# CogSP/CoEvoNet

Hardware: AMD Instinct MI355X
Metric: env-steps/sec (agent-steps of the whole job; generations/sec in gens_per_sec), Co-GA simple_adversary_v3 pop=200 HoF=5 (higher is better)
Workload: dtype f32

## Files before the change

### coevonet_amd/csrc/coevo_common.hip.h

```cpp
#pragma once
#include <hip/hip_runtime.h>
#include <stdint.h>

#include "../../include/coevo.h"

namespace coevo {

constexpr int H1 = COEVO_FC_H1;
constexpr int H2 = COEVO_FC_H2;
constexpr int NACT = COEVO_FC_NACT;
constexpr float LN_EPS = 1e-5f;

__host__ __device__ constexpr int64_t fc_off_b1(int D) { return (int64_t)D * H1; }
__host__ __device__ constexpr int64_t fc_off_w2(int D) { return fc_off_b1(D) + 3 * H1; }
__host__ __device__ constexpr int64_t fc_off_b2(int D) { return fc_off_w2(D) + (int64_t)H1 * H2; }
__host__ __device__ constexpr int64_t fc_off_w3(int D) { return fc_off_b2(D) + 3 * H2; }
__host__ __device__ constexpr int64_t fc_off_b3(int D) { return fc_off_w3(D) + NACT * H2; }
__host__ __device__ constexpr int64_t fc_params(int D) { return fc_off_b3(D) + NACT; }
__host__ __device__ constexpr int64_t fc_stride(int D) { return (fc_params(D) + 63) / 64 * 64; }
__host__ __device__ constexpr int64_t fc_off_g1(int D) { return fc_off_b1(D) + H1; }
__host__ __device__ constexpr int64_t fc_off_g2(int D) { return fc_off_b2(D) + H2; }
__host__ __device__ inline bool fc_slab_is_layernorm(int64_t s, int D)
{
    const int64_t g1 = fc_off_g1(D), g2 = fc_off_g2(D);
// ... 157 lines not shown
{
    const size_t N = (size_t)n;
    s.ax = st[0 * N + g]; s.ay = st[1 * N + g];
    s.bx = st[2 * N + g]; s.by = st[3 * N + g];
    s.cx = st[4 * N + g]; s.cy = st[5 * N + g];
    s.avx = st[6 * N + g]; s.avy = st[7 * N + g];
    s.bvx = st[8 * N + g]; s.bvy = st[9 * N + g];
    s.cvx = st[10 * N + g]; s.cvy = st[11 * N + g];
    s.l0x = st[12 * N + g]; s.l0y = st[13 * N + g];
    s.l1x = st[14 * N + g]; s.l1y = st[15 * N + g];
    s.gx = st[16 * N + g]; s.gy = st[17 * N + g];
}

__device__ __forceinline__ void mpe_store_game(double *st, int n, int g, const MpeGame &s)
{
    const size_t N = (size_t)n;
    st[0 * N + g] = s.ax; st[1 * N + g] = s.ay;
    st[2 * N + g] = s.bx; st[3 * N + g] = s.by;
    st[4 * N + g] = s.cx; st[5 * N + g] = s.cy;
    st[6 * N + g] = s.avx; st[7 * N + g] = s.avy;
    st[8 * N + g] = s.bvx; st[9 * N + g] = s.bvy;
    st[10 * N + g] = s.cvx; st[11 * N + g] = s.cvy;
    st[12 * N + g] = s.l0x; st[13 * N + g] = s.l0y;
    st[14 * N + g] = s.l1x; st[15 * N + g] = s.l1y;
    st[16 * N + g] = s.gx; st[17 * N + g] = s.gy;
}

__device__ __forceinline__ void mpe_move(double &pos, double &vel, double u, int pos_first)
{
    const double f = (((u * 5.0) + 0.0) / 1.0) * 0.1;
    if (pos_first) pos = pos + vel * 0.1;
    vel = vel * 0.75;
    vel = vel + f;
    if (!pos_first) pos = pos + vel * 0.1;
}

__device__ __forceinline__ double mpe_ux(int act) { return act == 1 ? -1.0 : (act == 2 ? 1.0 : 0.0); }
__device__ __forceinline__ double mpe_uy(int act) { return act == 3 ? -1.0 : (act == 4 ? 1.0 : 0.0); }

__device__ __forceinline__ void mpe_world_move(MpeGame &s, int act_a, int act_b, int act_c, int pos_first)
{
    mpe_move(s.ax, s.avx, mpe_ux(act_a), pos_first);
    mpe_move(s.ay, s.avy, mpe_uy(act_a), pos_first);
    mpe_move(s.bx, s.bvx, mpe_ux(act_b), pos_first);
    mpe_move(s.by, s.bvy, mpe_uy(act_b), pos_first);
    mpe_move(s.cx, s.cvx, mpe_ux(act_c), pos_first);
    mpe_move(s.cy, s.cvy, mpe_uy(act_c), pos_first);
}

__device__ __forceinline__ void mpe_world_step(MpeGame &s, int act_a, int act_b, int act_c, int pos_first,
                                               double &r_good, double &r_adv)
{
    mpe_world_move(s, act_a, act_b, act_c, pos_first);
    double dx = s.ax - s.gx, dy = s.ay - s.gy;
    const double da = sqrt(dx * dx + dy * dy);
    dx = s.bx - s.gx; dy = s.by - s.gy;
    const double db = sqrt(dx * dx + dy * dy);
    dx = s.cx - s.gx; dy = s.cy - s.gy;
    const double dc = sqrt(dx * dx + dy * dy);
    r_adv = -da;
    const double m = (dc < db) ? dc : db;
    r_good = -m + da;
}

__host__ __device__ __forceinline__ void mpe_obs_good(const MpeGame &s, double mex, double mey, double ox, double oy, float o[10])
{
    o[0] = (float)(s.gx - mex);  o[1] = (float)(s.gy - mey);
    o[2] = (float)(s.l0x - mex); o[3] = (float)(s.l0y - mey);
    o[4] = (float)(s.l1x - mex); o[5] = (float)(s.l1y - mey);
    o[6] = (float)(s.ax - mex);  o[7] = (float)(s.ay - mey);
    o[8] = (float)(ox - mex);    o[9] = (float)(oy - mey);
}

__host__ __device__ __forceinline__ void mpe_obs_from_game(const MpeGame &s, int slot, float o[10])
{
    if (slot == COEVO_SLOT_ADVERSARY) {
        o[0] = (float)(s.l0x - s.ax); o[1] = (float)(s.l0y - s.ay);
        o[2] = (float)(s.l1x - s.ax); o[3] = (float)(s.l1y - s.ay);
        o[4] = (float)(s.bx - s.ax);  o[5] = (float)(s.by - s.ay);
        o[6] = (float)(s.cx - s.ax);  o[7] = (float)(s.cy - s.ay);
        o[8] = 0.0f;                  o[9] = 0.0f;
    } else if (slot == COEVO_SLOT_AGENT_0) {
        mpe_obs_good(s, s.bx, s.by, s.cx, s.cy, o);
    } else {
        mpe_obs_good(s, s.cx, s.cy, s.bx, s.by, o);
    }
}

__device__ __forceinline__ void mpe_fused_observe(const double *st_prev, double *st_next, const int32_t *act_prev,
                                         const int32_t *game_limit, int n, int g, int slot, int cycle, int pos_first,
                                         float *obs_out)
{
    const size_t N = (size_t)n;
    MpeGame s;
    mpe_load_game(st_prev, n, g, s);
    if (cycle > 0) {
        const int limit = game_limit ? game_limit[g] : 0x7fffffff;
        const int t0 = 3 * (cycle - 1);
        const bool stepped = t0 + 2 < limit;
        double r_good = 0.0, r_adv = 0.0;
        if (stepped) {
            const int a0 = act_prev[3 * g], a1 = act_prev[3 * g + 1], a2 = act_prev[3 * g + 2];
            if (slot == COEVO_SLOT_ADVERSARY) mpe_world_step(s, a0, a1, a2, pos_first, r_good, r_adv);
            else mpe_world_move(s, a0, a1, a2, pos_first);
        }
        if (slot == COEVO_SLOT_ADVERSARY) {
            double rg_prev = st_prev[18 * N + g], a_adv = st_prev[19 * N + g], a_a0 = st_prev[20 * N + g],
                   a_a1 = st_prev[21 * N + g];
            if (t0 < limit) a_adv = a_adv + rg_prev;
            if (t0 + 1 < limit) a_a0 = a_a0 + rg_prev;
            if (stepped) { a_a1 = a_a1 + r_adv; rg_prev = r_good; }
            mpe_store_game(st_next, n, g, s);
            st_next[18 * N + g] = rg_prev;
            st_next[19 * N + g] = a_adv;
            st_next[20 * N + g] = a_a0;
            st_next[21 * N + g] = a_a1;
        }
    }
    mpe_obs_from_game(s, slot, obs_out);
}

__device__ inline double block_sum_f64(double v, double *scratch)
{
#pragma unroll
    for (int m = 1; m < 64; m <<= 1) v = v + __shfl_xor(v, m, 64);
    const int w = threadIdx.x >> 6;
    if ((threadIdx.x & 63) == 0) scratch[w] = v;
    __syncthreads();
    const double tot = ((scratch[0] + scratch[1]) + scratch[2]) + scratch[3];
    __syncthreads();
    return tot;
}

template <class DistOf>
__device__ inline double sharing_row_total(DistOf dist_of, int n, double *scratch)
{
    double s = 0.0;
    for (int i = threadIdx.x; i < n; i += 256) s += (double)dist_of(i);
    const float sigma = (float)(block_sum_f64(s, scratch) / (double)n);
    double sc = 0.0;
    for (int i = threadIdx.x; i < n; i += 256) {
        const float sh = 1.0f - dist_of(i) / sigma;
        if (!(sh <= 0.0f)) sc += (double)sh;
    }
    return block_sum_f64(sc, scratch);
}

__device__ inline float ga_fitness_value(double reward, int hof, float share)
{
    const float total = (float)(reward / (double)hof);
    return total / (1.0f + share);
}

__device__ __forceinline__ double wave_sum_partials(const double *partial, int n_blocks)
{
    double v = 0.0;
    for (int b = threadIdx.x; b < n_blocks; b += 64) v += partial[b];
#pragma unroll
    for (int m = 1; m < 64; m <<= 1) v = v + __shfl_xor(v, m, 64);
    return v;
}

__device__ inline bool bad_post_relu(float y) { return __builtin_isnan(y) || (__builtin_isinf(y) && y > 0.0f); }
__device__ inline float relu_keep_nan(float y) { return !(y <= 0.0f) ? y : 0.0f; }

}

#ifndef COEVO_TU_FLAGS
#define COEVO_TU_FLAGS ""
#endif
#define COEVO_DEFINE_TU_FLAGS(tu) \
    namespace coevo { const char *tu_flags_##tu() { return COEVO_TU_FLAGS; } }

#define COEVO_HIP_CHECK(expr)                        \
    do {                                             \
        hipError_t _e = (expr);                      \
        if (_e != hipSuccess) return COEVO_ERR_HIP;  \
    } while (0)
```

### coevonet_amd/csrc/mpe_env.hip

```cpp
#include "coevo_common.hip.h"

#include "../../include/coevo_crossplay.h"

namespace coevo {

typedef unsigned __int128 u128;

__host__ __device__ inline u128 pcg_mult()
{
    return (((u128)0x2360ED051FC65DA4ULL) << 64) | (u128)0x4385DF649FCCF645ULL;
}

__host__ __device__ inline uint64_t pcg_output(u128 s)
{
    const uint64_t hi = (uint64_t)(s >> 64), lo = (uint64_t)s;
    const uint64_t x = hi ^ lo;
    const unsigned r = (unsigned)(hi >> 58);
    return (x >> r) | (x << ((64 - r) & 63));
}

__host__ __device__ inline u128 pcg_advance(u128 state, u128 inc, u128 delta)
{
    u128 acc_mult = 1, acc_plus = 0, cur_mult = pcg_mult(), cur_plus = inc;
    while (delta > 0) {
        if (delta & 1) {
            acc_mult *= cur_mult;
            acc_plus = acc_plus * cur_mult + cur_plus;
        }
        cur_plus = (cur_mult + 1) * cur_plus;
        cur_mult *= cur_mult;
        delta >>= 1;
    }
    return acc_mult * state + acc_plus;
}

__host__ __device__ __forceinline__ void mpe_reset_game(double *st, int n, int g, coevo_pcg64 rng, uint64_t ordinal);

__global__ void mpe_reset_kernel(double *st, int n, int game_first, int count, coevo_pcg64 rng,
                                 int64_t first_ordinal, const int32_t *gen_dev, int64_t ordinals_per_gen, int unsigned_first)
{
    const int i = blockIdx.x * blockDim.x + threadIdx.x;
    if (i >= count) return;
    int64_t first = first_ordinal + (gen_dev ? (int64_t)(*gen_dev) * ordinals_per_gen : 0);
    if (first < 0 && !unsigned_first) first = 0;
    mpe_reset_game(st, n, game_first + i, rng, (uint64_t)first + (uint64_t)i);
}

__global__ void mpe_reset_episodes_kernel(double *st, int n, int game_first, int count, coevo_pcg64 rng,
                                          uint64_t first_ordinal, int episodes)
{
    const int i = blockIdx.x * blockDim.x + threadIdx.x;
    if (i >= count) return;
    mpe_reset_game(st, n, game_first + i, rng, first_ordinal + (uint64_t)(i % episodes));
}

static_assert(sizeof(coevo_reset_seg) == 16, "layout mirrored by coevonet_amd/lib.py ResetSeg");
struct ResetSegs { coevo_reset_seg s[COEVO_MAX_JOBS]; };
__global__ void mpe_reset_multi_kernel(double *st, int n, ResetSegs segs, coevo_pcg64 rng, uint64_t *stamps, int n_stamps,
                                       int32_t *zero_words, int n_zero)
{
    const coevo_reset_seg &sg = segs.s[blockIdx.y];
    const int i = blockIdx.x * blockDim.x + threadIdx.x;
    if (zero_words && blockIdx.y == gridDim.y - 1)
        for (int j = i; j < n_zero; j += gridDim.x * blockDim.x) zero_words[j] = 0;
    if (stamps && blockIdx.y == 0)
        for (int j = i; j < n_stamps; j += gridDim.x * blockDim.x) {
            stamps[2 * j] = ~0ull;
            stamps[2 * j + 1] = 0ull;
        }
    if (i >= sg.count) return;
    mpe_reset_game(st, n, sg.game_first + i, rng, sg.first_ordinal + (uint64_t)i);
}

__host__ __device__ __forceinline__ void mpe_reset_game(double *st, int n, int g, coevo_pcg64 rng, uint64_t ordinal)
{
    const u128 inc = ((u128)rng.pcg_inc_hi << 64) | rng.pcg_inc_lo;
    u128 s = ((u128)rng.pcg_state_hi << 64) | rng.pcg_state_lo;
    s = pcg_advance(s, inc, (u128)(ordinal >> 1) * 21);
    s = s * pcg_mult() + inc;
    const uint64_t c = pcg_output(s);
    const uint32_t half = (ordinal & 1) ? (uint32_t)(c >> 32) : (uint32_t)c;
    const int goal = (int)(((uint64_t)half * 2) >> 32);
    if (ordinal & 1) s = pcg_advance(s, inc, 10);
    double d[10];
#pragma unroll
    for (int i = 0; i < 10; ++i) {
        s = s * pcg_mult() + inc;
        d[i] = -1.0 + 2.0 * ((double)(pcg_output(s) >> 11) * (1.0 / 9007199254740992.0));
    }
    const size_t N = (size_t)n;
#pragma unroll
    for (int i = 0; i < 6; ++i) {
        st[i * N + g] = d[i];
        st[(6 + i) * N + g] = 0.0;
    }
#pragma unroll
    for (int i = 0; i < 4; ++i) st[(12 + i) * N + g] = d[6 + i];
    st[16 * N + g] = d[6 + 2 * goal];
    st[17 * N + g] = d[7 + 2 * goal];
    st[18 * N + g] = 0.0;
    st[19 * N + g] = 0.0;
    st[20 * N + g] = 0.0;
    st[21 * N + g] = 0.0;
    st[22 * N + g] = (double)goal;
    st[23 * N + g] = 0.0;
}

__host__ __device__ inline float mpe_observe_at(const double *st, int n, const int32_t *row_game, const int32_t *row_slot, int i)
{
    const int row = i / COEVO_OBS_STRIDE, k = i % COEVO_OBS_STRIDE;
    const int slot = row_slot[row];
    const int D = (slot == COEVO_SLOT_ADVERSARY) ? 8 : 10;
    return (k < D) ? mpe_obs_element(st, n, row_game[row], slot, k) : 0.0f;
}

__global__ void mpe_observe_kernel(const double *st, int n, const int32_t *row_game, const int32_t *row_slot,
                                   int n_rows, float *obs)
{
    const int i = blockIdx.x * blockDim.x + threadIdx.x;
    if (i >= n_rows * COEVO_OBS_STRIDE) return;
    obs[i] = mpe_observe_at(st, n, row_game, row_slot, i);
}

__host__ __device__ inline void mpe_step_game(double *st, int n, const int32_t *game_rows, const int32_t *actions,
                                              int cycle, const int32_t *game_limit, int pos_first, int g)
{
    const size_t N = (size_t)n;
    const int limit = game_limit ? game_limit[g] : 0x7fffffff;
    const int t0 = 3 * cycle;
    if (t0 >= limit) return;
    const double rg_prev = st[18 * N + g];
    st[19 * N + g] = st[19 * N + g] + rg_prev;
    if (t0 + 1 < limit) st[20 * N + g] = st[20 * N + g] + rg_prev;
    if (t0 + 2 >= limit) return;
    double d[3];
    const double gx = st[16 * N + g], gy = st[17 * N + g];
#pragma unroll
    for (int i = 0; i < 3; ++i) {
        const int act = actions[game_rows[3 * g + i]];
        double u[2] = {0.0, 0.0};
        if (act == 1) u[0] = -1.0;
        if (act == 2) u[0] = +1.0;
        if (act == 3) u[1] = -1.0;
        if (act == 4) u[1] = +1.0;
        double p[2];
#pragma unroll
        for (int c = 0; c < 2; ++c) {
            const double f = (((u[c] * 5.0) + 0.0) / 1.0) * 0.1;
            double pos = st[(2 * i + c) * N + g], vel = st[(6 + 2 * i + c) * N + g];
            if (pos_first) pos = pos + vel * 0.1;
            vel = vel * 0.75;
            vel = vel + f;
            if (!pos_first) pos = pos + vel * 0.1;
            st[(2 * i + c) * N + g] = pos;
            st[(6 + 2 * i + c) * N + g] = vel;
            p[c] = pos;
        }
        const double dx = p[0] - gx, dy = p[1] - gy;
        d[i] = sqrt(dx * dx + dy * dy);
    }
    const double r_adv = -d[0];
    const double m = (d[2] < d[1]) ? d[2] : d[1];
    const double r_good = -m + d[0];
    st[21 * N + g] = st[21 * N + g] + r_adv;
    st[18 * N + g] = r_good;
}

__global__ void mpe_step_kernel(double *st, int n, const int32_t *game_rows, const int32_t *actions, int cycle,
                                const int32_t *game_limit, int pos_first)
{
    const int g = blockIdx.x * blockDim.x + threadIdx.x;
    if (g < n) mpe_step_game(st, n, game_rows, actions, cycle, game_limit, pos_first, g);
}

typedef coevo_final_pack FinalPack;
static_assert(sizeof(coevo_final_pack) == 40, "layout mirrored by coevonet_amd/lib.py FinalPack");

__global__ void mpe_final_step_kernel(const double *st, int n, const int32_t *act, int cycle,
                                      const int32_t *game_limit, int pos_first, double *rewards, FinalPack pk)
{
    const int g = blockIdx.x * blockDim.x + threadIdx.x;
    if (g >= n) return;
    const size_t N = (size_t)n;
    double a_adv = st[19 * N + g], a_a0 = st[20 * N + g], a_a1 = st[21 * N + g];
    if (cycle >= 0) {
        const int limit = game_limit ? game_limit[g] : 0x7fffffff;
        const int t0 = 3 * cycle;
        const double rg_prev = st[18 * N + g];
        if (t0 < limit) a_adv = a_adv + rg_prev;
        if (t0 + 1 < limit) a_a0 = a_a0 + rg_prev;
        if (t0 + 2 < limit) {
            MpeGame s;
            mpe_load_game(st, n, g, s);
            double r_good, r_adv;
            mpe_world_step(s, act[3 * g], act[3 * g + 1], act[3 * g + 2], pos_first, r_good, r_adv);
            a_a1 = a_a1 + r_adv;
        }
    }
    rewards[3 * (size_t)g + 0] = a_a0;
    rewards[3 * (size_t)g + 1] = a_a1;
    rewards[3 * (size_t)g + 2] = a_adv;
    if (pk.out && g < pk.n_roles * pk.n_local * pk.hof && g % pk.hof == pk.hof - 1) {
        const int ij = g / pk.hof, role = ij / pk.n_local, j = ij % pk.n_local;
        double *o = pk.out + 4 * (size_t)ij;
        o[0] = a_a0;
        o[1] = a_a1;
        o[2] = a_adv;
        o[3] = (double)pk.dist[(size_t)role * pk.dist_pitch + pk.dist_first + j];
    }
}

__global__ void mpe_rewards_kernel(const double *st, int n, double *rewards)
{
    const int g = blockIdx.x * blockDim.x + threadIdx.x;
    if (g >= n) return;
    const size_t N = (size_t)n;
    rewards[3 * (size_t)g + 0] = st[20 * N + g];
    rewards[3 * (size_t)g + 1] = st[21 * N + g];
    rewards[3 * (size_t)g + 2] = st[19 * N + g];
}

}

extern "C" int coevo_mpe_reset_gen(double *state, int n_games, int game_first, int count, coevo_pcg64 rng,
                                   int64_t first_ordinal, const int32_t *gen_dev, int64_t ordinals_per_gen,
                                   void *stream)
{
    if (!state || n_games <= 0 || game_first < 0 || count < 0 || game_first + count > n_games) return COEVO_ERR_ARG;
    if (count == 0) return COEVO_OK;
    hipLaunchKernelGGL(coevo::mpe_reset_kernel, dim3((count + 127) / 128), dim3(128), 0, (hipStream_t)stream,
                       state, n_games, game_first, count, rng, first_ordinal, gen_dev, ordinals_per_gen, 0);
    COEVO_HIP_CHECK(hipGetLastError());
    return COEVO_OK;
}

static int reset_multi_launch(double *state, int n_games, const coevo_reset_seg *segs, int n_segs, coevo_pcg64 rng,
// ... 242 lines not shown
```

### coevonet_amd/csrc/select.hip

```cpp
#include "coevo_common.hip.h"
#include <stdio.h>

namespace coevo {

__global__ __launch_bounds__(256) void fc_distance_kernel(const float *ref_net, const float *pop_slab, int D,
                                                           float *dist)
{
    __shared__ double scratch[4];
    const int64_t stride = fc_stride(D), P = fc_params(D);
    const int64_t g1 = fc_off_g1(D), g2 = fc_off_g2(D);
    const float *wi = pop_slab + (int64_t)blockIdx.x * stride;
    double acc = 0.0;
    for (int64_t s0 = (int64_t)threadIdx.x * 4; s0 < stride; s0 += 1024) {
        const float4 a = *reinterpret_cast<const float4 *>(wi + s0);
        const float4 b = *reinterpret_cast<const float4 *>(ref_net + s0);
        const float av[4] = {a.x, a.y, a.z, a.w}, bv[4] = {b.x, b.y, b.z, b.w};
#pragma unroll
        for (int c = 0; c < 4; ++c) {
            const int64_t s = s0 + c;
            const bool ln = (s >= g1 && s < g1 + 2 * H1) || (s >= g2 && s < g2 + 2 * H2);
            if (s < P && !ln) {
                const float d = av[c] - bv[c];
                acc += (double)d * (double)d;
            }
        }
    }
    const double tot = block_sum_f64(acc, scratch);
    if (threadIdx.x == 0) dist[blockIdx.x] = (float)sqrt(tot);
}

__global__ __launch_bounds__(64) void dist_finalize_kernel(const double *partial, int n_blocks, float *dist, int first,
                                                            const float *head)
{
    const int c = blockIdx.x;
    const double v = wave_sum_partials(partial + (size_t)c * n_blocks, n_blocks);
    if (threadIdx.x == 0) {
        dist[first + c] = (float)sqrt(v);
        if (c == 0 && head) dist[first - 1] = *head;
    }
}

static_assert(sizeof(coevo_fc_finalize_job) == 40, "layout mirrored by coevonet_amd/lib.py FinalizeJob");
struct FinalizeJobs { coevo_fc_finalize_job j[COEVO_MAX_JOBS]; };
__global__ __launch_bounds__(64) void dist_finalize_multi_kernel(FinalizeJobs jobs, int32_t *tick)
{
    const coevo_fc_finalize_job &jb = jobs.j[blockIdx.y];
    const int c = blockIdx.x, l = threadIdx.x;
    if (tick && blockIdx.x == 0 && blockIdx.y == 0 && l == 0) *tick += 1;
    if (c >= jb.n) return;
    const double v = wave_sum_partials(jb.dist_partial + (size_t)c * jb.n_blocks, jb.n_blocks);
    if (l == 0) {
        jb.dist[jb.first + c] = (float)sqrt(v);
        if (c == 0 && jb.head) jb.dist[jb.first - 1] = *jb.head;
    }
}

__global__ void gather_f32_kernel(float *dst, const float *src, const int32_t *idx, int n)
{
    const int i = blockIdx.x * blockDim.x + threadIdx.x;
    if (i < n) dst[i] = src[idx[i]];
}

__global__ __launch_bounds__(256) void sharing_score_kernel(const float *dist, int n, float *score)
{
    __shared__ double scratch[4];
    const double tot = sharing_row_total([&](int i) { return dist[i]; }, n, scratch);
    if (threadIdx.x == 0) *score = (float)tot;
}

__global__ void ga_fitness_kernel(const double *rewards, int game_first, int pop, int games_per_individual,
                                  int hof, int slot, const float *diversity, float *fitness)
{
    const int i = blockIdx.x * blockDim.x + threadIdx.x;
    if (i >= pop) return;
    const int gpi = games_per_individual;
    const double last = rewards[3 * (size_t)(game_first + i * gpi + gpi - 1) + slot];
    fitness[i] = ga_fitness_value(last, hof, *diversity);
}

__device__ inline bool rank_less(float a, int ia, float b, int ib)
{
    const bool an = __builtin_isnan(a), bn = __builtin_isnan(b);
    if (an || bn) return (!an && bn) || (an && bn && ia < ib);
    return (a < b) || (a == b && ia < ib);
}

__global__ __launch_bounds__(256) void rank_desc_kernel(const float *fitness, int n, int32_t *order)
{
    __shared__ float f[4096];
    for (int i = threadIdx.x; i < n; i += 256) f[i] = fitness[i];
    __syncthreads();
    for (int i = threadIdx.x; i < n; i += 256) {
        const float fi = f[i];
        int rank = 0;
        for (int j = 0; j < n; ++j) rank += rank_less(f[j], j, fi, i) ? 1 : 0;
        order[n - 1 - rank] = i;
    }
}

struct GaSelectArgs {
    coevo_ga_select_role role[3];
    int pop, games_per_individual, hof;
    const double *gathered;
    int n_local, n_roles;
    coevo_ga_adapt_args adapt;
    int with_adapt, n_roles_launched;
};

static_assert(sizeof(coevo_ga_adapt_args) == 88, "layout mirrored by coevonet_amd/lib.py GaAdaptArgs");
__device__ inline void ga_adapt_body(const coevo_ga_adapt_args &a);

__global__ __launch_bounds__(256) void ga_select_kernel(GaSelectArgs a)
{
    __shared__ double scratch[4];
    __shared__ float f[4096];
    __shared__ float div_s;
    if ((int)blockIdx.x >= a.n_roles_launched) {
        if (a.with_adapt && blockIdx.y == 0 && threadIdx.x == 0) ga_adapt_body(a.adapt);
        return;
    }
    const coevo_ga_select_role R = a.role[blockIdx.x];
    const int n = a.pop;
    const bool first_slice = blockIdx.y == 0;
    auto rec = [&](int i) {
        return a.gathered + 4 * ((size_t)((i / a.n_local) * a.n_roles + (int)blockIdx.x) * a.n_local + i % a.n_local);
    };
    auto dist_of = [&](int i) { return a.gathered ? (float)rec(i)[3] : R.dist[i]; };
    const double tot = sharing_row_total(dist_of, n, scratch);
    if (threadIdx.x == 0) {
        div_s = (float)tot;
        if (first_slice) *R.diversity = (float)tot;
    }
    __syncthreads();
    const int gpi = a.games_per_individual;
    for (int i = threadIdx.x; i < n; i += 256) {
        const double last = a.gathered ? rec(i)[R.slot] : R.rewards[3 * (size_t)(R.game_first + i * gpi + gpi - 1) + R.slot];
        const float fit = ga_fitness_value(last, a.hof, div_s);
        f[i] = fit;
        if (first_slice) R.fitness[i] = fit;
    }
    __syncthreads();
    const int i = blockIdx.y * 256 + threadIdx.x;
    if (i < n) {
        const float fi = f[i];
        int rank = 0;
        for (int j = 0; j < n; ++j) rank += rank_less(f[j], j, fi, i) ? 1 : 0;
        R.order[n - 1 - rank] = i;
        if (rank == n - 1 && R.best_dist) *R.best_dist = dist_of(i);
    }
}

__device__ inline double np_mean_le10(const double *a, int n)
{
    double res;
    if (n < 8) {
        res = 0.0;
        for (int i = 0; i < n; ++i) res += a[i];
    } else {
        res = ((a[0] + a[1]) + (a[2] + a[3])) + ((a[4] + a[5]) + (a[6] + a[7]));
        for (int i = 8; i < n; ++i) res += a[i];
    }
    return res / (double)n;
}

__device__ inline void ga_adapt_body(const coevo_ga_adapt_args &a)
{
    const double *rewards = a.rewards;
    double *hist = a.hist, *sig_hist = a.sig_hist, *sigma64 = a.sigma64;
    const int cap = a.cap, eval_first = a.eval_first_game;
    const int g = *a.gen_dev;
    if (a.sigma32_prev)
        for (int s = 0; s < 3; ++s) a.sigma32_prev[s] = a.sigma32[s];
    if (g > 0 && g - 1 < cap) {
        const int e = g - 1;
        for (int s = 0; s < 3; ++s) {
            double tot = 0.0;
            for (int i = 0; i < 10; ++i) tot += rewards[3 * (size_t)(eval_first + i) + s];
            hist[(size_t)s * cap + e] = tot / 10;
        }
        if (a.adaptive) {
            bool worse[3];
            for (int s = 0; s < 3; ++s) {
                const double *h = hist + (size_t)s * cap;
                const int len = e + 1;
                if (e > 10) {
                    const int n_old = (len >= 20) ? 10 : len - 10;
                    const double m_new = np_mean_le10(h + len - 10, 10);
                    const double m_old = np_mean_le10(h + (len >= 20 ? len - 20 : 0), n_old);
                    worse[s] = m_new < m_old;
                } else {
                    worse[s] = false;
                }
            }
            const double s1_before = sigma64[1];
            sigma64[0] = worse[0] ? fmin(s1_before * 1.2, a.sig_max) : fmax(sigma64[0] * 0.95, a.sig_min);
            sigma64[1] = worse[1] ? fmin(sigma64[1] * 1.2, a.sig_max) : fmax(sigma64[1] * 0.95, a.sig_min);
            sigma64[2] = worse[2] ? fmin(sigma64[2] * 1.2, a.sig_max) : fmax(sigma64[2] * 0.95, a.sig_min);
        }
        for (int s = 0; s < 3; ++s) sig_hist[(size_t)s * cap + e] = sigma64[s];
    }
    for (int s = 0; s < 3; ++s) a.sigma32[s] = (float)sigma64[s];
}

__global__ void ga_adapt_kernel(coevo_ga_adapt_args a)
{
    if (threadIdx.x != 0 || blockIdx.x != 0) return;
    ga_adapt_body(a);
}

__global__ __launch_bounds__(256) void centered_rank_kernel(const float *f, int n, float *out)
{
    const int i = blockIdx.x * 256 + threadIdx.x;
    if (i >= n) return;
    const float fi = f[i];
    int rank = 0;
    for (int j = 0; j < n; ++j) rank += rank_less(f[j], j, fi, i) ? 1 : 0;
    out[i] = (n > 1) ? (float)rank / (float)(n - 1) - 0.5f : 0.0f;
}

__global__ void counter_add_kernel(int32_t *p, int v) { if (threadIdx.x == 0 && blockIdx.x == 0) *p += v; }

}

using namespace coevo;

extern "C" int coevo_ga_adapt_sigma(const double *rewards, int eval_first_game, const int32_t *gen_dev, double *hist,
                                    double *sig_hist, int cap, double *sigma64, float *sigma32, double sig_min,
                                    double sig_max, int adaptive, void *stream)
{
    if (!rewards || !gen_dev || !hist || !sig_hist || !sigma64 || !sigma32 || cap <= 0 || eval_first_game < 0)
        return COEVO_ERR_ARG;
    const coevo_ga_adapt_args a{rewards, gen_dev, hist, sig_hist, sigma64, sigma32, nullptr, sig_min, sig_max, eval_first_game,
                                cap, adaptive, 0};
    hipLaunchKernelGGL(ga_adapt_kernel, dim3(1), dim3(64), 0, (hipStream_t)stream, a);
    COEVO_HIP_CHECK(hipGetLastError());
    return COEVO_OK;
}

extern "C" int coevo_centered_ranks(const float *fitness, int n, float *out, void *stream)
{
    if (!fitness || !out || n <= 0 || fitness == out) return COEVO_ERR_ARG;
    hipLaunchKernelGGL(centered_rank_kernel, dim3((n + 255) / 256), dim3(256), 0, (hipStream_t)stream, fitness, n, out);
    COEVO_HIP_CHECK(hipGetLastError());
    return COEVO_OK;
}

extern "C" int coevo_counter_add(int32_t *counter, int value, void *stream)
{
    if (!counter) return COEVO_ERR_ARG;
    hipLaunchKernelGGL(counter_add_kernel, dim3(1), dim3(64), 0, (hipStream_t)stream, counter, value);
    COEVO_HIP_CHECK(hipGetLastError());
    return COEVO_OK;
}

extern "C" int coevo_fc_diversity(const float *ref_net, const float *pop_slab, int n, int D, float *dist,
                                  float *score, void *stream)
{
    if (!ref_net || !pop_slab || !dist || !score || n <= 0 || !fc_dim_ok(D)) return COEVO_ERR_ARG;
    hipLaunchKernelGGL(fc_distance_kernel, dim3(n), dim3(256), 0, (hipStream_t)stream, ref_net, pop_slab, D, dist);
    hipLaunchKernelGGL(sharing_score_kernel, dim3(1), dim3(256), 0, (hipStream_t)stream, dist, n, score);
    COEVO_HIP_CHECK(hipGetLastError());
    return COEVO_OK;
}

extern "C" int coevo_fc_distance(const float *ref_net, const float *pop_slab, int n, int D, float *dist, void *stream)
{
    if (!ref_net || !pop_slab || !dist || n <= 0 || !fc_dim_ok(D)) return COEVO_ERR_ARG;
    hipLaunchKernelGGL(fc_distance_kernel, dim3(n), dim3(256), 0, (hipStream_t)stream, ref_net, pop_slab, D, dist);
    COEVO_HIP_CHECK(hipGetLastError());
    return COEVO_OK;
}

extern "C" int coevo_fc_distance_finalize(const double *partial, int n_blocks, int n, float *dist, int first,
                                          const float *head, void *stream)
{
    if (!partial || !dist || n_blocks <= 0 || n <= 0 || first < 0 || (head && first < 1)) return COEVO_ERR_ARG;
    hipLaunchKernelGGL(dist_finalize_kernel, dim3(n), dim3(64), 0, (hipStream_t)stream, partial, n_blocks, dist, first,
                       head);
    COEVO_HIP_CHECK(hipGetLastError());
    return COEVO_OK;
}

static int finalize_multi_launch(const coevo_fc_finalize_job *jobs, int n_jobs, int32_t *tick, void *stream)
{
    if (!jobs || n_jobs < 1 || n_jobs > COEVO_MAX_JOBS) return COEVO_ERR_ARG;
    FinalizeJobs fj{};
    int nmax = 0;
    for (int i = 0; i < n_jobs; ++i) {
        const coevo_fc_finalize_job &j = jobs[i];
        if (!j.dist_partial || !j.dist || j.n_blocks <= 0 || j.n < 0 || j.first < 0 || (j.head && j.first < 1)) return COEVO_ERR_ARG;
        fj.j[i] = j;
        nmax = j.n > nmax ? j.n : nmax;
    }
    if (nmax == 0 && !tick) return COEVO_OK;
    hipLaunchKernelGGL(dist_finalize_multi_kernel, dim3(nmax > 0 ? nmax : 1, n_jobs), dim3(64), 0, (hipStream_t)stream, fj, tick);
    COEVO_HIP_CHECK(hipGetLastError());
    return COEVO_OK;
}

extern "C" int coevo_fc_distance_finalize_multi(const coevo_fc_finalize_job *jobs, int n_jobs, void *stream)
{
    return finalize_multi_launch(jobs, n_jobs, nullptr, stream);
}

extern "C" int coevo_fc_distance_finalize_multi_tick(const coevo_fc_finalize_job *jobs, int n_jobs, int32_t *counter, void *stream)
{
    if (!counter) return COEVO_ERR_ARG;
    return finalize_multi_launch(jobs, n_jobs, counter, stream);
}

extern "C" int coevo_gather_f32(float *dst, const float *src, const int32_t *idx, int n, void *stream)
{
    if (!dst || !src || !idx || n <= 0) return COEVO_ERR_ARG;
    hipLaunchKernelGGL(gather_f32_kernel, dim3((n + 127) / 128), dim3(128), 0, (hipStream_t)stream, dst, src, idx, n);
    COEVO_HIP_CHECK(hipGetLastError());
    return COEVO_OK;
}

extern "C" int coevo_sharing_score(const float *dist, int n, float *score, void *stream)
{
    if (!dist || !score || n <= 0) return COEVO_ERR_ARG;
    hipLaunchKernelGGL(sharing_score_kernel, dim3(1), dim3(256), 0, (hipStream_t)stream, dist, n, score);
    COEVO_HIP_CHECK(hipGetLastError());
    return COEVO_OK;
}

extern "C" int coevo_ga_fitness(const double *rewards, int game_first, int pop, int games_per_individual, int hof,
                                int slot, const float *diversity, float *fitness, void *stream)
{
    if (!rewards || !diversity || !fitness || pop <= 0 || hof <= 0 || games_per_individual <= 0 || slot < 0 ||
        slot > 2 || game_first < 0)
        return COEVO_ERR_ARG;
    hipLaunchKernelGGL(ga_fitness_kernel, dim3((pop + 127) / 128), dim3(128), 0, (hipStream_t)stream, rewards,
                       game_first, pop, games_per_individual, hof, slot, diversity, fitness);
    COEVO_HIP_CHECK(hipGetLastError());
    return COEVO_OK;
}

extern "C" int coevo_rank_desc(const float *fitness, int n, int32_t *order, void *stream)
{
    if (!fitness || !order || n <= 0 || n > 4096) return COEVO_ERR_ARG;
    hipLaunchKernelGGL(rank_desc_kernel, dim3(1), dim3(256), 0, (hipStream_t)stream, fitness, n, order);
    COEVO_HIP_CHECK(hipGetLastError());
    return COEVO_OK;
}

static int ga_select_launch(const coevo_ga_select_role *roles, int n_roles, int pop, int games_per_individual, int hof,
                            const double *gathered, int n_local, const coevo_ga_adapt_args *adapt, void *stream)
{
    if (!roles || n_roles < 1 || n_roles > 3 || pop <= 0 || pop > 4096 || hof <= 0 || games_per_individual <= 0)
        return COEVO_ERR_ARG;
    coevo::GaSelectArgs a{};
    for (int r = 0; r < n_roles; ++r) {
        const coevo_ga_select_role &R = roles[r];
        if ((!gathered && (!R.dist || !R.rewards)) || !R.diversity || !R.fitness || !R.order || R.slot < 0 || R.slot > 2 ||
            R.game_first < 0)
            return COEVO_ERR_ARG;
        a.role[r] = R;
    }
    a.gathered = gathered; a.n_local = n_local; a.n_roles = n_roles;
    a.pop = pop; a.games_per_individual = games_per_individual; a.hof = hof;
    a.n_roles_launched = n_roles;
    if (adapt) { a.adapt = *adapt; a.with_adapt = 1; }
    hipLaunchKernelGGL(coevo::ga_select_kernel, dim3(n_roles + (adapt ? 1 : 0), (pop + 255) / 256), dim3(256), 0,
                       (hipStream_t)stream, a);
    COEVO_HIP_CHECK(hipGetLastError());
    return COEVO_OK;
}

extern "C" int coevo_ga_select(const coevo_ga_select_role *roles, int n_roles, int pop, int games_per_individual,
                               int hof, void *stream)
{
    return ga_select_launch(roles, n_roles, pop, games_per_individual, hof, nullptr, 0, nullptr, stream);
}

extern "C" int coevo_ga_select_adapt(const coevo_ga_select_role *roles, int n_roles, int pop, int games_per_individual, int hof,
                                     const double *gathered, int n_local, const coevo_ga_adapt_args *adapt, void *stream)
{
    if (!adapt || !adapt->rewards || !adapt->gen_dev || !adapt->hist || !adapt->sig_hist || !adapt->sigma64 || !adapt->sigma32 ||
        adapt->cap <= 0 || adapt->eval_first_game < 0)
        return COEVO_ERR_ARG;
    if (gathered && (n_local <= 0 || pop % n_local)) return COEVO_ERR_ARG;
    return ga_select_launch(roles, n_roles, pop, gathered ? 1 : games_per_individual, hof, gathered, n_local, adapt, stream);
}

extern "C" int coevo_ga_select_gathered(const coevo_ga_select_role *roles, int n_roles, int pop, int hof,
                                        const double *gathered, int n_local, void *stream)
{
    if (!gathered || n_local <= 0 || pop % n_local) return COEVO_ERR_ARG;
    return ga_select_launch(roles, n_roles, pop, 1, hof, gathered, n_local, nullptr, stream);
}

extern "C" int coevo_version(void) { return COEVO_VERSION; }

COEVO_DEFINE_TU_FLAGS(select)
namespace coevo {
const char *tu_flags_fc_forward(); const char *tu_flags_mpe_env(); const char *tu_flags_offspring();
const char *tu_flags_rollout_api(); const char *tu_flags_deepqn(); const char *tu_flags_dqn_engine();
const char *tu_flags_host_rollout(); const char *tu_flags_host_placement();
}

extern "C" const char *coevo_build_flags(void)
{
    static char buf[1024];
    static bool done = false;
    if (!done) {
        const char *names[] = {"fc_forward", "mpe_env", "offspring", "select", "rollout_api", "deepqn", "dqn_engine", "host_rollout",
                               "host_placement"};
        const char *flags[] = {coevo::tu_flags_fc_forward(), coevo::tu_flags_mpe_env(), coevo::tu_flags_offspring(),
                               coevo::tu_flags_select(), coevo::tu_flags_rollout_api(), coevo::tu_flags_deepqn(),
                               coevo::tu_flags_dqn_engine(), coevo::tu_flags_host_rollout(), coevo::tu_flags_host_placement()};
        size_t n = 0;
        buf[0] = 0;
        for (int i = 0; i < 9; ++i) {
            if (!flags[i][0]) continue;
            const int w = snprintf(buf + n, sizeof(buf) - n, "%s%s: %s", n ? "; " : "", names[i], flags[i]);
            if (w < 0 || (size_t)w >= sizeof(buf) - n) break;
            n += (size_t)w;
        }
        done = true;
    }
    return buf;
}
```

Baseline: 154.3 million.

## Speed up PCG jumps, distance finalize, rank compare, and sigma adaptation

Adds a precomputed constant table of PCG multiplier and increment powers so device-side resets jump with a table lookup per bit instead of squaring 128-bit values in a loop. It also packs four wavefronts into each distance-finalize block and unrolls the partial-sum loads, makes the rank comparison branchless, prefetches the last-game reward before the sharing reduction, and parallelises the sigma-adaptation loads across threads via LDS. These target latency in several small kernels. The cost is a 4KB constant table and more complex code across many unrelated spots.

```diff
diff --git a/coevonet_amd/csrc/coevo_common.hip.h b/coevonet_amd/csrc/coevo_common.hip.h
--- a/coevonet_amd/csrc/coevo_common.hip.h
+++ b/coevonet_amd/csrc/coevo_common.hip.h
@@ -333,14 +333,22 @@
     return total / (1.0f + share);
 }
 
-__device__ __forceinline__ double wave_sum_partials(const double *partial, int n_blocks)
+__device__ __forceinline__ double wave_sum_partials(const double *partial, int n_blocks, int lane)
 {
     double v = 0.0;
-    for (int b = threadIdx.x; b < n_blocks; b += 64) v += partial[b];
+    for (int b = lane; b < n_blocks; b += 256) {
+        double p[4];
+#pragma unroll
+        for (int k = 0; k < 4; ++k) p[k] = (b + 64 * k < n_blocks) ? partial[b + 64 * k] : 0.0;
+#pragma unroll
+        for (int k = 0; k < 4; ++k)
+            if (b + 64 * k < n_blocks) v += p[k];
+    }
 #pragma unroll
     for (int m = 1; m < 64; m <<= 1) v = v + __shfl_xor(v, m, 64);
     return v;
 }
+__device__ __forceinline__ double wave_sum_partials(const double *partial, int n_blocks) { return wave_sum_partials(partial, n_blocks, (int)threadIdx.x); }
 
 __device__ inline bool bad_post_relu(float y) { return __builtin_isnan(y) || (__builtin_isinf(y) && y > 0.0f); }
 __device__ inline float relu_keep_nan(float y) { return !(y <= 0.0f) ? y : 0.0f; }
diff --git a/coevonet_amd/csrc/mpe_env.hip b/coevonet_amd/csrc/mpe_env.hip
--- a/coevonet_amd/csrc/mpe_env.hip
+++ b/coevonet_amd/csrc/mpe_env.hip
@@ -1,38 +1,9 @@
 #include "coevo_common.hip.h"
+#include "pcg64_jump.hip.h"
 
 #include "../../include/coevo_crossplay.h"
 
 namespace coevo {
-
-typedef unsigned __int128 u128;
-
-__host__ __device__ inline u128 pcg_mult()
-{
-    return (((u128)0x2360ED051FC65DA4ULL) << 64) | (u128)0x4385DF649FCCF645ULL;
-}
-
-__host__ __device__ inline uint64_t pcg_output(u128 s)
-{
-    const uint64_t hi = (uint64_t)(s >> 64), lo = (uint64_t)s;
-    const uint64_t x = hi ^ lo;
-    const unsigned r = (unsigned)(hi >> 58);
-    return (x >> r) | (x << ((64 - r) & 63));
-}
-
-__host__ __device__ inline u128 pcg_advance(u128 state, u128 inc, u128 delta)
-{
-    u128 acc_mult = 1, acc_plus = 0, cur_mult = pcg_mult(), cur_plus = inc;
-    while (delta > 0) {
-        if (delta & 1) {
-            acc_mult *= cur_mult;
-            acc_plus = acc_plus * cur_mult + cur_plus;
-        }
-        cur_plus = (cur_mult + 1) * cur_plus;
-        cur_mult *= cur_mult;
-        delta >>= 1;
-    }
-    return acc_mult * state + acc_plus;
-}
 
 __host__ __device__ __forceinline__ void mpe_reset_game(double *st, int n, int g, coevo_pcg64 rng, uint64_t ordinal);
 
@@ -76,12 +47,20 @@
 {
     const u128 inc = ((u128)rng.pcg_inc_hi << 64) | rng.pcg_inc_lo;
     u128 s = ((u128)rng.pcg_state_hi << 64) | rng.pcg_state_lo;
+#ifdef __HIP_DEVICE_COMPILE__
+    s = pcg_jump(s, inc, (u128)(ordinal >> 1) * 21);
+#else
     s = pcg_advance(s, inc, (u128)(ordinal >> 1) * 21);
+#endif
     s = s * pcg_mult() + inc;
     const uint64_t c = pcg_output(s);
     const uint32_t half = (ordinal & 1) ? (uint32_t)(c >> 32) : (uint32_t)c;
     const int goal = (int)(((uint64_t)half * 2) >> 32);
+#ifdef __HIP_DEVICE_COMPILE__
+    if (ordinal & 1) s = pcg_jump_pow2<1>(pcg_jump_pow2<3>(s, inc), inc);
+#else
     if (ordinal & 1) s = pcg_advance(s, inc, 10);
+#endif
     double d[10];
 #pragma unroll
     for (int i = 0; i < 10; ++i) {
diff --git a/coevonet_amd/csrc/pcg64_jump.hip.h b/coevonet_amd/csrc/pcg64_jump.hip.h
--- /dev/null
+++ b/coevonet_amd/csrc/pcg64_jump.hip.h
@@ -0,0 +1,94 @@
+#pragma once
+#include <stdint.h>
+
+#ifdef __HIPCC__
+#define COEVO_HD __host__ __device__
+#else
+#define COEVO_HD
+#endif
+
+namespace coevo {
+
+typedef unsigned __int128 u128;
+
+COEVO_HD constexpr u128 pcg_mult()
+{
+    return (((u128)0x2360ED051FC65DA4ULL) << 64) | (u128)0x4385DF649FCCF645ULL;
+}
+
+COEVO_HD inline uint64_t pcg_output(u128 s)
+{
+    const uint64_t hi = (uint64_t)(s >> 64), lo = (uint64_t)s;
+    const uint64_t x = hi ^ lo;
+    const unsigned r = (unsigned)(hi >> 58);
+    return (x >> r) | (x << ((64 - r) & 63));
+}
+
+COEVO_HD inline u128 pcg_advance(u128 state, u128 inc, u128 delta)
+{
+    u128 acc_mult = 1, acc_plus = 0, cur_mult = pcg_mult(), cur_plus = inc;
+    while (delta > 0) {
+        if (delta & 1) {
+            acc_mult *= cur_mult;
+            acc_plus = acc_plus * cur_mult + cur_plus;
+        }
+        cur_plus = (cur_mult + 1) * cur_plus;
+        cur_mult *= cur_mult;
+        delta >>= 1;
+    }
+    return acc_mult * state + acc_plus;
+}
+
+struct PcgPowers {
+    uint64_t a[128][2], g[128][2];
+};
+
+constexpr PcgPowers pcg_make_powers()
+{
+    PcgPowers t{};
+    u128 a = pcg_mult(), g = 1;
+    for (int b = 0; b < 128; ++b) {
+        t.a[b][0] = (uint64_t)a;
+        t.a[b][1] = (uint64_t)(a >> 64);
+        t.g[b][0] = (uint64_t)g;
+        t.g[b][1] = (uint64_t)(g >> 64);
+        g *= a + 1;
+        a *= a;
+    }
+    return t;
+}
+
+constexpr PcgPowers pcg_powers_host = pcg_make_powers();
+#ifdef __HIPCC__
+__constant__ const PcgPowers pcg_powers_dev = pcg_make_powers();
+#endif
+
+COEVO_HD inline const PcgPowers &pcg_powers()
+{
+#ifdef __HIP_DEVICE_COMPILE__
+    return pcg_powers_dev;
+#else
+    return pcg_powers_host;
+#endif
+}
+
+template <int B>
+COEVO_HD inline u128 pcg_jump_pow2(u128 s, u128 inc)
+{
+    constexpr PcgPowers t = pcg_make_powers();
+    constexpr u128 a = ((u128)t.a[B][1] << 64) | t.a[B][0], g = ((u128)t.g[B][1] << 64) | t.g[B][0];
+    return a * s + g * inc;
+}
+
+COEVO_HD inline u128 pcg_jump(u128 s, u128 inc, u128 delta)
+{
+    const PcgPowers &t = pcg_powers();
+    for (int b = 0; b < 128 && (delta >> b) != 0; ++b) {
+        const u128 a = ((u128)t.a[b][1] << 64) | t.a[b][0], g = ((u128)t.g[b][1] << 64) | t.g[b][0];
+        const u128 plus = g * inc;
+        if ((delta >> b) & 1) s = a * s + plus;
+    }
+    return s;
+}
+
+}
diff --git a/coevonet_amd/csrc/select.hip b/coevonet_amd/csrc/select.hip
--- a/coevonet_amd/csrc/select.hip
+++ b/coevonet_amd/csrc/select.hip
@@ -42,13 +42,14 @@
 
 static_assert(sizeof(coevo_fc_finalize_job) == 40, "layout mirrored by coevonet_amd/lib.py FinalizeJob");
 struct FinalizeJobs { coevo_fc_finalize_job j[COEVO_MAX_JOBS]; };
-__global__ __launch_bounds__(64) void dist_finalize_multi_kernel(FinalizeJobs jobs, int32_t *tick)
+constexpr int FINALIZE_WAVES = 4;
+__global__ __launch_bounds__(64 * FINALIZE_WAVES) void dist_finalize_multi_kernel(FinalizeJobs jobs, int32_t *tick)
 {
     const coevo_fc_finalize_job &jb = jobs.j[blockIdx.y];
-    const int c = blockIdx.x, l = threadIdx.x;
-    if (tick && blockIdx.x == 0 && blockIdx.y == 0 && l == 0) *tick += 1;
+    const int c = blockIdx.x * FINALIZE_WAVES + (int)(threadIdx.x >> 6), l = threadIdx.x & 63;
+    if (tick && blockIdx.x == 0 && blockIdx.y == 0 && threadIdx.x == 0) *tick += 1;
     if (c >= jb.n) return;
-    const double v = wave_sum_partials(jb.dist_partial + (size_t)c * jb.n_blocks, jb.n_blocks);
+    const double v = wave_sum_partials(jb.dist_partial + (size_t)c * jb.n_blocks, jb.n_blocks, l);
     if (l == 0) {
         jb.dist[jb.first + c] = (float)sqrt(v);
         if (c == 0 && jb.head) jb.dist[jb.first - 1] = *jb.head;
@@ -81,8 +82,7 @@
 __device__ inline bool rank_less(float a, int ia, float b, int ib)
 {
     const bool an = __builtin_isnan(a), bn = __builtin_isnan(b);
-    if (an || bn) return (!an && bn) || (an && bn && ia < ib);
-    return (a < b) || (a == b && ia < ib);
+    return (a < b) | (!an & bn) | (((a == b) | (an & bn)) & (ia < ib));
 }
 
 __global__ __launch_bounds__(256) void rank_desc_kernel(const float *fitness, int n, int32_t *order)
@@ -108,15 +108,17 @@
 };
 
 static_assert(sizeof(coevo_ga_adapt_args) == 88, "layout mirrored by coevonet_amd/lib.py GaAdaptArgs");
-__device__ inline void ga_adapt_body(const coevo_ga_adapt_args &a);
+constexpr int ADAPT_LDS_DOUBLES = 92;
+__device__ inline void ga_adapt_body(const coevo_ga_adapt_args &a, double *lds);
 
 __global__ __launch_bounds__(256) void ga_select_kernel(GaSelectArgs a)
 {
     __shared__ double scratch[4];
-    __shared__ float f[4096];
+    __shared__ __attribute__((aligned(8))) float f[4096];
     __shared__ float div_s;
+    static_assert(sizeof(f) >= ADAPT_LDS_DOUBLES * sizeof(double), "the sigma rule's block keeps its values where the roles' blocks keep f");
     if ((int)blockIdx.x >= a.n_roles_launched) {
-        if (a.with_adapt && blockIdx.y == 0 && threadIdx.x == 0) ga_adapt_body(a.adapt);
+        if (a.with_adapt && blockIdx.y == 0) ga_adapt_body(a.adapt, reinterpret_cast<double *>(f));
         return;
     }
     const coevo_ga_select_role R = a.role[blockIdx.x];
@@ -126,15 +128,19 @@
         return a.gathered + 4 * ((size_t)((i / a.n_local) * a.n_roles + (int)blockIdx.x) * a.n_local + i % a.n_local);
     };
     auto dist_of = [&](int i) { return a.gathered ? (float)rec(i)[3] : R.dist[i]; };
+    const int gpi = a.games_per_individual;
+    auto reward_of = [&](int i) {
+        return a.gathered ? rec(i)[R.slot] : R.rewards[3 * (size_t)(R.game_first + i * gpi + gpi - 1) + R.slot];
+    };
+    const double last0 = ((int)threadIdx.x < n) ? reward_of(threadIdx.x) : 0.0;
     const double tot = sharing_row_total(dist_of, n, scratch);
     if (threadIdx.x == 0) {
         div_s = (float)tot;
         if (first_slice) *R.diversity = (float)tot;
     }
     __syncthreads();
-    const int gpi = a.games_per_individual;
     for (int i = threadIdx.x; i < n; i += 256) {
-        const double last = a.gathered ? rec(i)[R.slot] : R.rewards[3 * (size_t)(R.game_first + i * gpi + gpi - 1) + R.slot];
+        const double last = (i == (int)threadIdx.x) ? last0 : reward_of(i);
         const float fit = ga_fitness_value(last, a.hof, div_s);
         f[i] = fit;
         if (first_slice) R.fitness[i] = fit;
@@ -163,49 +169,67 @@
     return res / (double)n;
 }
 
-__device__ inline void ga_adapt_body(const coevo_ga_adapt_args &a)
-{
-    const double *rewards = a.rewards;
+__device__ inline void ga_adapt_body(const coevo_ga_adapt_args &a, double *lds)
+{
     double *hist = a.hist, *sig_hist = a.sig_hist, *sigma64 = a.sigma64;
-    const int cap = a.cap, eval_first = a.eval_first_game;
+    const int cap = a.cap, t = threadIdx.x;
     const int g = *a.gen_dev;
+    const bool record = g > 0 && g - 1 < cap;
+    const int e = g - 1, len = g;
+    double *rw = lds, *hh = lds + 32;
+    double r = 0.0, h = 0.0, sg[3] = {0.0, 0.0, 0.0};
+    float s32[3] = {0.0f, 0.0f, 0.0f};
+    if (record && t < 30) r = a.rewards[3 * (size_t)(a.eval_first_game + t % 10) + t / 10];
+    if (record && a.adaptive && t < 60) {
+        const int pos = len - 20 + t % 20;
+        if (pos >= 0 && pos < e) h = hist[(size_t)(t / 20) * cap + pos];
+    }
+    if (t == 0) {
+        for (int s = 0; s < 3; ++s) sg[s] = sigma64[s];
+        if (a.sigma32_prev)
+            for (int s = 0; s < 3; ++s) s32[s] = a.sigma32[s];
+    }
+    if (t < 30) rw[t] = r;
+    if (t < 60) hh[t] = h;
+    __syncthreads();
+    if (t != 0) return;
     if (a.sigma32_prev)
-        for (int s = 0; s < 3; ++s) a.sigma32_prev[s] = a.sigma32[s];
-    if (g > 0 && g - 1 < cap) {
-        const int e = g - 1;
+        for (int s = 0; s < 3; ++s) a.sigma32_prev[s] = s32[s];
+    if (record) {
         for (int s = 0; s < 3; ++s) {
             double tot = 0.0;
-            for (int i = 0; i < 10; ++i) tot += rewards[3 * (size_t)(eval_first + i) + s];
-            hist[(size_t)s * cap + e] = tot / 10;
+            for (int i = 0; i < 10; ++i) tot += rw[10 * s + i];
+            hh[20 * s + 19] = hist[(size_t)s * cap + e] = tot / 10;
         }
         if (a.adaptive) {
             bool worse[3];
             for (int s = 0; s < 3; ++s) {
-                const double *h = hist + (size_t)s * cap;
-                const int len = e + 1;
+                const double *hs = hh + 20 * s;
                 if (e > 10) {
                     const int n_old = (len >= 20) ? 10 : len - 10;
-                    const double m_new = np_mean_le10(h + len - 10, 10);
-                    const double m_old = np_mean_le10(h + (len >= 20 ? len - 20 : 0), n_old);
+                    const double m_new = np_mean_le10(hs + 10, 10);
+                    const double m_old = np_mean_le10(hs + (len >= 20 ? 0 : 20 - len), n_old);
                     worse[s] = m_new < m_old;
                 } else {
                     worse[s] = false;
                 }
             }
-            const double s1_before = sigma64[1];
-            sigma64[0] = worse[0] ? fmin(s1_before * 1.2, a.sig_max) : fmax(sigma64[0] * 0.95, a.sig_min);
-            sigma64[1] = worse[1] ? fmin(sigma64[1] * 1.2, a.sig_max) : fmax(sigma64[1] * 0.95, a.sig_min);
-            sigma64[2] = worse[2] ? fmin(sigma64[2] * 1.2, a.sig_max) : fmax(sigma64[2] * 0.95, a.sig_min);
+            const double s1_before = sg[1];
+            sg[0] = worse[0] ? fmin(s1_before * 1.2, a.sig_max) : fmax(sg[0] * 0.95, a.sig_min);
+            sg[1] = worse[1] ? fmin(sg[1] * 1.2, a.sig_max) : fmax(sg[1] * 0.95, a.sig_min);
+            sg[2] = worse[2] ? fmin(sg[2] * 1.2, a.sig_max) : fmax(sg[2] * 0.95, a.sig_min);
+            for (int s = 0; s < 3; ++s) sigma64[s] = sg[s];
         }
-        for (int s = 0; s < 3; ++s) sig_hist[(size_t)s * cap + e] = sigma64[s];
-    }
-    for (int s = 0; s < 3; ++s) a.sigma32[s] = (float)sigma64[s];
-}
-
-__global__ void ga_adapt_kernel(coevo_ga_adapt_args a)
-{
-    if (threadIdx.x != 0 || blockIdx.x != 0) return;
-    ga_adapt_body(a);
+        for (int s = 0; s < 3; ++s) sig_hist[(size_t)s * cap + e] = sg[s];
+    }
+    for (int s = 0; s < 3; ++s) a.sigma32[s] = (float)sg[s];
+}
+
+__global__ __launch_bounds__(64) void ga_adapt_kernel(coevo_ga_adapt_args a)
+{
+    __shared__ double lds[ADAPT_LDS_DOUBLES];
+    if (blockIdx.x != 0) return;
+    ga_adapt_body(a, lds);
 }
 
 __global__ __launch_bounds__(256) void centered_rank_kernel(const float *f, int n, float *out)
@@ -293,7 +317,8 @@
         nmax = j.n > nmax ? j.n : nmax;
     }
     if (nmax == 0 && !tick) return COEVO_OK;
-    hipLaunchKernelGGL(dist_finalize_multi_kernel, dim3(nmax > 0 ? nmax : 1, n_jobs), dim3(64), 0, (hipStream_t)stream, fj, tick);
+    hipLaunchKernelGGL(dist_finalize_multi_kernel, dim3(nmax > 0 ? (nmax + FINALIZE_WAVES - 1) / FINALIZE_WAVES : 1, n_jobs),
+                       dim3(64 * FINALIZE_WAVES), 0, (hipStream_t)stream, fj, tick);
     COEVO_HIP_CHECK(hipGetLastError());
     return COEVO_OK;
 }
```

Measured after the change: 154.7 million, median of 2. Within noise of the previous version (+0.2%).
